# adityabalu/DiffNet

Hardware: AMD Instinct MI355X
Metric: elements*gauss_pts/sec (FEM loss+grad) (higher is better)
Workload: dtype f32; 1 GPU; 2-D Poisson energy loss + gradient wrt u, Q1, 512^2 nodes, 3^2 Gauss pts, batch 64/GPU, nu+f nodal fields, Dirichlet mask on all boundary faces held as one bit per node and sample (a general mask array), fused single pass (BASELINE.json configs[1] mesh); every step evaluates the next of 4 different batches in rotation (nu, f and the mask stream from HBM with non-temporal loads; of the 4 x 67 MB of; batch_per_gpu=64, parallelism=batch-sharded x1, batches_in_rotation=4, mask_format=bits

## Files before the change

diffnet_amd/csrc/dn_common.h:

```cpp
#pragma once
#include <hip/hip_runtime.h>
#include <stdint.h>

#include "../../include/diffnet_hip.h"

#define DN_WAVE 64

#define DN_LAUNCH_CHECK()                         \
    do {                                          \
        hipError_t e__ = hipGetLastError();       \
        if (e__ != hipSuccess) return (int)e__;   \
    } while (0)

namespace dn {

enum ConfigKey : int { CFG_PLAN2D = 0, CFG_PLAN3D, CFG_PLAN_FSDT, CFG_Q1_RULE_KERNEL, CFG_GPE_GATHER, CFG_GPE_TILED, CFG_Q1_3D_T16, CFG_Q1_3D_E1SUM, CFG_FSDT_GENERIC, CFG_Q1_3D_E1, CFG_HANDOVER_SPIN_LIMIT, CFG_CONV2D_V1, CFG_CONV_WRW_WGS, CFG_Q1_3D_N2, CFG_FSDT_FORM, CFG_COUNT };
const char* config(ConfigKey k);

__device__ __forceinline__ double wave_sum(double v) {
#pragma unroll
    for (int off = DN_WAVE / 2; off > 0; off >>= 1) v += __shfl_down(v, off, DN_WAVE);
    return v;
}

__device__ __forceinline__ double block_sum(double v, double* scratch, int tid, int nthreads) {
    v = wave_sum(v);
    const int lane = tid & (DN_WAVE - 1), wave = tid / DN_WAVE;
    if (lane == 0) scratch[wave] = v;
    __syncthreads();
    double r = 0.0;
    if (tid == 0) {
        const int nw = (nthreads + DN_WAVE - 1) / DN_WAVE;
        for (int w = 0; w < nw; ++w) r += scratch[w];
    }
    __syncthreads();
    return r;
}

__device__ __forceinline__ void block_sum2(double& a, double& b, double* scratch, int tid, int nthreads) {
    a = wave_sum(a);
    b = wave_sum(b);
    const int lane = tid & (DN_WAVE - 1), wave = tid / DN_WAVE;
    const int nw = (nthreads + DN_WAVE - 1) / DN_WAVE;
    if (lane == 0) { scratch[wave] = a; scratch[nw + wave] = b; }
    __syncthreads();
    double ra = 0.0, rb = 0.0;
    if (tid == 0) {
        for (int w = 0; w < nw; ++w) { ra += scratch[w]; rb += scratch[nw + w]; }
    }
    __syncthreads();
    a = ra; b = rb;
}

template <int N>
struct VecT;
template <>
struct VecT<1> { using type = float; };
template <>
struct VecT<2> { using type = float2; };
template <>
struct VecT<4> { using type = float4; };

#ifndef DN_NT_STORES
#define DN_NT_STORES 0
#endif
template <typename V, typename T>
__device__ __forceinline__ V ld_at(const T* __restrict__ base, unsigned index) {
    return *reinterpret_cast<const V*>(reinterpret_cast<const char*>(base) + (index * (unsigned)sizeof(T)));
}
template <typename V, typename T>
__device__ __forceinline__ void st_at(T* __restrict__ base, unsigned index, const V& v) {
#if DN_NT_STORES
    char* a = reinterpret_cast<char*>(base) + (index * (unsigned)sizeof(T));
    if constexpr (sizeof(V) == 16) {
        typedef float v4f __attribute__((ext_vector_type(4)));
        __builtin_nontemporal_store(__builtin_bit_cast(v4f, v), reinterpret_cast<v4f*>(a));
    } else if constexpr (sizeof(V) == 8) {
        typedef float v2f __attribute__((ext_vector_type(2)));
        __builtin_nontemporal_store(__builtin_bit_cast(v2f, v), reinterpret_cast<v2f*>(a));
    } else {
        __builtin_nontemporal_store(v, reinterpret_cast<V*>(a));
    }
#else
    *reinterpret_cast<V*>(reinterpret_cast<char*>(base) + (index * (unsigned)sizeof(T))) = v;
#endif
}

template <int NW, bool VEC, typename T>
__device__ __forceinline__ void load_seg(const T* __restrict__ base, unsigned rowoff, int x0, int nx, T (&dst)[NW + 1]) {
    if constexpr (VEC && (NW == 2 || NW == 4)) {
        const unsigned xl = (unsigned)min(x0, nx - NW);
        if constexpr (sizeof(T) == 4) {
            using V = typename VecT<NW>::type;
            const V v = ld_at<V>(base, rowoff + xl);
            const T* vf = reinterpret_cast<const T*>(&v);
#pragma unroll
            for (int k = 0; k < NW; ++k) dst[k] = vf[k];
        } else {
            static_assert(sizeof(T) == 1, "load_seg: 1- or 4-byte elements");
            if constexpr (NW == 4) {
                const uint32_t w = ld_at<uint32_t>(base, rowoff + xl);
#pragma unroll
                for (int k = 0; k < 4; ++k) dst[k] = (T)((w >> (8 * k)) & 0xffu);
            } else {
                const uint16_t w = ld_at<uint16_t>(base, rowoff + xl);
                dst[0] = (T)(w & 0xffu);
                dst[1] = (T)(w >> 8);
            }
        }
    } else {
#pragma unroll
        for (int k = 0; k < NW; ++k) dst[k] = ld_at<T>(base, rowoff + (unsigned)min(x0 + k, nx - 1));
    }
    dst[NW] = ld_at<T>(base, rowoff + (unsigned)min(x0 + NW, nx - 1));
}

template <int NW, bool VEC, typename T>
__device__ __forceinline__ void load_seg_stream(const T* __restrict__ base, unsigned rowoff, int x0, int nx, T (&dst)[NW + 1]) {
    if constexpr (VEC && NW == 4 && sizeof(T) == 4) {
        typedef T v4t __attribute__((ext_vector_type(4)));
        const unsigned xl = (unsigned)min(x0, nx - NW);
        const v4t v = __builtin_nontemporal_load(reinterpret_cast<const v4t*>(reinterpret_cast<const char*>(base) + (rowoff + xl) * 4u));
        dst[0] = v.x; dst[1] = v.y; dst[2] = v.z; dst[3] = v.w;
        dst[NW] = ld_at<T>(base, rowoff + (unsigned)min(x0 + NW, nx - 1));
    } else if constexpr (VEC && NW == 4 && sizeof(T) == 1) {
        const unsigned xl = (unsigned)min(x0, nx - NW);
        const uint32_t w = __builtin_nontemporal_load(reinterpret_cast<const uint32_t*>(reinterpret_cast<const char*>(base) + (rowoff + xl)));
#pragma unroll
        for (int k = 0; k < 4; ++k) dst[k] = (T)((w >> (8 * k)) & 0xffu);
        dst[NW] = ld_at<T>(base, rowoff + (unsigned)min(x0 + NW, nx - 1));
    } else {
        load_seg<NW, VEC>(base, rowoff, x0, nx, dst);
    }
}

template <int NW, bool VEC, typename T>
__device__ __forceinline__ void load_own(const T* __restrict__ base, unsigned rowoff, int x0, int nx, T (&dst)[NW]) {
    if constexpr (VEC && (NW == 2 || NW == 4)) {
        const unsigned xl = (unsigned)min(x0, nx - NW);
        if constexpr (sizeof(T) == 4) {
            using V = typename VecT<NW>::type;
            const V v = ld_at<V>(base, rowoff + xl);
            const T* vf = reinterpret_cast<const T*>(&v);
#pragma unroll
            for (int k = 0; k < NW; ++k) dst[k] = vf[k];
        } else {
            if constexpr (NW == 4) {
                const uint32_t w = ld_at<uint32_t>(base, rowoff + xl);
#pragma unroll
                for (int k = 0; k < 4; ++k) dst[k] = (T)((w >> (8 * k)) & 0xffu);
            } else {
                const uint16_t w = ld_at<uint16_t>(base, rowoff + xl);
                dst[0] = (T)(w & 0xffu);
                dst[1] = (T)(w >> 8);
            }
        }
    } else {
#pragma unroll
        for (int k = 0; k < NW; ++k) dst[k] = ld_at<T>(base, rowoff + (unsigned)min(x0 + k, nx - 1));
    }
}

template <int NW, bool VEC>
__device__ __forceinline__ void store_seg(float* __restrict__ base, unsigned rowoff, int x0, int nx, const float (&src)[NW]) {
    if constexpr (VEC && (NW == 2 || NW == 4)) {
        if (x0 + NW <= nx) {
            using V = typename VecT<NW>::type;
            V v;
            float* vf = reinterpret_cast<float*>(&v);
#pragma unroll
            for (int k = 0; k < NW; ++k) vf[k] = src[k];
            st_at<V>(base, rowoff + (unsigned)x0, v);
        }
    } else {
#pragma unroll
        for (int k = 0; k < NW; ++k)
            if (x0 + k < nx) st_at<float>(base, rowoff + (unsigned)(x0 + k), src[k]);
    }
}

}
```

diffnet_amd/csrc/poisson2d_q1_cf.hip:

```cpp
#include <cstdlib>
#include <type_traits>

#define DN_NT_STORES 1
#include "poisson_common.h"

namespace dn {

enum : int { CF_NU = 1, CF_F = 2, CF_BC = 8, CF_BC_U8C = 16, CF_BC_PACKED = 32, CF_PK_NB1 = 64, CF_PK_NB2 = 128, CF_UA = 256, CF_ONE = 512 };

template <int E>
struct CfRow {
    float u[E + 1], n[E + 1], f[E + 1];
    float g[E + 1];
    float du[E], pn[E];
    float keep[E];
    float keepx;
    BcRaw<E> bc;
    uint32_t m8[2][2];
    uint32_t mb[2];
    uint32_t bx[2];
};

constexpr int CF_W = 4;
constexpr int CF_TS = 128;
constexpr int CF_NSLOT = 64;
constexpr unsigned CF_SPIN_MAX = 1u << 20;

__device__ __forceinline__ unsigned lds_addr(const void* p) { return (unsigned)(uintptr_t)(__attribute__((address_space(3))) const void*)p; }
__device__ __forceinline__ void lds_st(unsigned a, float v) { asm volatile("ds_write_b32 %0, %1" ::"v"(a), "v"(v) : "memory"); }
__device__ __forceinline__ void lds_st(unsigned a, unsigned v) { asm volatile("ds_write_b32 %0, %1" ::"v"(a), "v"(v) : "memory"); }
__device__ __forceinline__ void lds_ld_nowait(float& d, unsigned a) { asm volatile("ds_read_b32 %0, %1" : "=v"(d) : "v"(a) : "memory"); }
__device__ __forceinline__ unsigned lds_ld_u(unsigned a) {
    unsigned d;
    asm volatile("ds_read_b32 %0, %1\n\ts_waitcnt lgkmcnt(0)" : "=v"(d) : "v"(a) : "memory");
    return d;
}
__device__ __forceinline__ float lds_ld(unsigned a) {
    float d;
    asm volatile("ds_read_b32 %0, %1\n\ts_waitcnt lgkmcnt(0)" : "=v"(d) : "v"(a) : "memory");
    return d;
}
template <int N>
__device__ __forceinline__ void lds_wait(float (&v)[N]) {
    if constexpr (N == 5) asm volatile("s_waitcnt lgkmcnt(0)" : "+v"(v[0]), "+v"(v[1]), "+v"(v[2]), "+v"(v[3]), "+v"(v[4])::"memory");
    else if constexpr (N == 4) asm volatile("s_waitcnt lgkmcnt(0)" : "+v"(v[0]), "+v"(v[1]), "+v"(v[2]), "+v"(v[3])::"memory");
    else if constexpr (N == 3) asm volatile("s_waitcnt lgkmcnt(0)" : "+v"(v[0]), "+v"(v[1]), "+v"(v[2])::"memory");
    else if constexpr (N == 2) asm volatile("s_waitcnt lgkmcnt(0)" : "+v"(v[0]), "+v"(v[1])::"memory");
    else { static_assert(N == 1, "lds_wait: 1..5 values"); asm volatile("s_waitcnt lgkmcnt(0)" : "+v"(v[0])::"memory"); }
}

template <int E, bool VEC, int FL, int W>
__global__ void __launch_bounds__(W > 1 ? CF_TS * W : 256, W > 1 ? 4 : 2) poisson2d_q1_cf_kernel(const PoissonParams p) {
    constexpr int NW = E;
    constexpr bool HAS_NU = (FL & CF_NU) != 0, HAS_F = (FL & CF_F) != 0;
    constexpr bool BC_ANY = (FL & (CF_BC | CF_BC_U8C | CF_BC_PACKED)) != 0, BC_U8C = (FL & CF_BC_U8C) != 0, BC_PACKED = (FL & CF_BC_PACKED) != 0;
    constexpr bool UA = (FL & CF_UA) != 0, ONE = (FL & CF_ONE) != 0;
    static_assert(!ONE || ((BC_PACKED || BC_U8C) && (FL & CF_PK_NB2) == 0), "CF_ONE: one packed or uint8-constant condition");
    static_assert(!UA || (E == 4 && VEC && W == 1), "CF_UA: four elements per thread, vector accesses, one strip per workgroup");
    const int T = W > 1 ? CF_TS : (int)blockDim.x;
    const int sub = W > 1 ? __builtin_amdgcn_readfirstlane((int)threadIdx.x / CF_TS) : 0;
    const int tid = W > 1 ? (int)threadIdx.x - sub * CF_TS : (int)threadIdx.x;
    const int chunk = blockIdx.x, strip = W > 1 ? (int)blockIdx.y * W + sub : selected_strip(p, (int)blockIdx.y), b = blockIdx.z;
    const bool active = W == 1 || strip < p.nstrips;
    const bool chain_dn = W > 1 && sub > 0;
    const bool chain_up = W > 1 && sub + 1 < W && strip + 1 < p.nstrips;
    const int q = chunk * (T - 1) + tid;
    const int ex0 = q * E;
    const int x0 = ex0;
    const bool col_owner = !(chunk > 0 && tid == 0);
    const bool lastcol = UA && x0 + NW == p.nx - 1;
    const int64_t nps = (int64_t)p.nx * p.ny;
    const SampleBases sb = sample_bases(p, b, nps);
    const int R = p.rows_per_strip;
    const int sb0 = strip * R, sc0 = min(sb0 + R, p.nely);
    const int ey_begin = (sb0 > 0 && !chain_dn) ? sb0 - 1 : sb0;
    const int ey_end = sc0;
    const int r_from = sb0;
    const int e_from = sb0, e_until = p.nely;
    const bool top_row = sc0 == p.nely;

    __shared__ float xch[2][256];
    __shared__ double red[W > 1 ? 4 * W : 8];
    __shared__ int last_flag;
    constexpr int CW = W > 1 ? W : 2, SEAM_WORDS = 6 * (E + 1);
    __shared__ float cf_edge[W > 1 ? W : 1][W > 1 ? CF_NSLOT : 1];
    __shared__ unsigned cf_xflag[W > 1 ? W : 1];
    __shared__ float cf_seam[CW - 1][W > 1 ? SEAM_WORDS : 1][W > 1 ? CF_TS : 1];
    __shared__ unsigned cf_sflag[CW - 1][2][2];
    const int lane = tid & 63, wv = __builtin_amdgcn_readfirstlane(tid >> 6);
    unsigned seq = 0u;
    if constexpr (W > 1) {
        static_assert(CF_TS == 128, "two waves per sub-strip");
        if (threadIdx.x < (unsigned)W) cf_xflag[threadIdx.x] = 0u;
        if (threadIdx.x < 4u * (W - 1)) (&cf_sflag[0][0][0])[threadIdx.x] = 0u;
        __syncthreads();
    }
    if ((blockIdx.x | blockIdx.y | blockIdx.z) == 0u) fold_prev_sums(p, (int)threadIdx.x, (int)blockDim.x, red);
    float spin_poison = 0.f;
    auto spin_until = [&](const unsigned* flag, unsigned want) {
        const unsigned fa = lds_addr(flag);
        const unsigned lim = p.spin_limit > 0 ? (unsigned)p.spin_limit : CF_SPIN_MAX;
        unsigned n = 0;
        for (; n < lim; ++n) {
            if ((unsigned)__builtin_amdgcn_readfirstlane((int)lds_ld_u(fa)) >= want) break;
            __builtin_amdgcn_s_sleep(1);
        }
        if (n == lim) spin_poison = __builtin_nanf("");
    };

    const bool has_mask[2] = {sb.mask[0] != nullptr, sb.mask[1] != nullptr};
    const uint8_t* mask8[2];
    mask8[0] = reinterpret_cast<const uint8_t*>(has_mask[0] ? sb.mask[0] : sb.mask[1]);
    mask8[1] = reinterpret_cast<const uint8_t*>(has_mask[1] ? sb.mask[1] : sb.mask[0]);

    constexpr unsigned NBITS = (1u << (NW + 1)) - 1u;
    constexpr int NB = !BC_PACKED ? 0 : ((FL & CF_PK_NB2) ? 2 : ((FL & CF_PK_NB1) ? 1 : 0));
    const bool isbits[2] = {p.bc[0].kind == DN_MASK_BITS, p.bc[1].kind == DN_MASK_BITS};
    const unsigned bsel[2] = {isbits[0] ? NBITS : 0u, isbits[1] ? NBITS : 0u};
    const int src0 = (NB == 2 || isbits[0]) ? 0 : 1;
    const int kone = p.bc[0].kind >= 0 ? 0 : 1;
    const uint32_t* bptr[2] = {reinterpret_cast<const uint32_t*>(sb.mask[src0]), reinterpret_cast<const uint32_t*>(sb.mask[1])};
    const unsigned brow[2] = {(unsigned)p.bc[src0].row_bytes / 4u, (unsigned)p.bc[1].row_bytes / 4u};
    unsigned bw0[2], bw1[2];
#pragma unroll
    for (int j = 0; j < 2; ++j) {
        const int rw = max((int)brow[j], 1);
        bw0[j] = (unsigned)min(x0 >> 5, rw - 1);
        bw1[j] = (unsigned)min((x0 >> 5) + 1, rw - 1);
    }
    const unsigned bsh = (unsigned)x0 & 31u;
    unsigned boxx[2] = {0u, 0u};
#pragma unroll
    for (int k = 0; k < 2; ++k) {
        const int faces = p.bc[k].kind == DN_MASK_BOX ? p.bc[k].box_faces : 0;
#pragma unroll
        for (int n = 0; n <= NW; ++n) {
            const bool on = ((faces & DN_FACE_XLO) && x0 + n == 0) || ((faces & DN_FACE_XHI) && x0 + n == p.nx - 1);
            boxx[k] |= on ? (1u << n) : 0u;
        }
    }
    const int ylo[2] = {(p.bc[0].kind == DN_MASK_BOX && (p.bc[0].box_faces & DN_FACE_YLO)) ? 0 : -1,
                        (p.bc[1].kind == DN_MASK_BOX && (p.bc[1].box_faces & DN_FACE_YLO)) ? 0 : -1};
    const int yhi[2] = {(p.bc[0].kind == DN_MASK_BOX && (p.bc[0].box_faces & DN_FACE_YHI)) ? p.ny - 1 : -1,
                        (p.bc[1].kind == DN_MASK_BOX && (p.bc[1].box_faces & DN_FACE_YHI)) ? p.ny - 1 : -1};
    auto packed_issue = [&](int yc, CfRow<E>& r) {
#pragma unroll
        for (int j = 0; j < NB; ++j) {
            const unsigned ro = (unsigned)yc * brow[j];
            const uint32_t w0 = ld_at<uint32_t>(bptr[j], ro + bw0[j]), w1 = ld_at<uint32_t>(bptr[j], ro + bw1[j]);
            r.mb[j] = __builtin_amdgcn_alignbit(w1, w0, bsh);
        }
        if constexpr (ONE) {
            if constexpr (NB == 0) r.bx[0] = (yc == (kone ? ylo[1] : ylo[0]) || yc == (kone ? yhi[1] : yhi[0])) ? NBITS : (kone ? boxx[1] : boxx[0]);
        } else {
#pragma unroll
            for (int k = 0; k < 2; ++k) r.bx[k] = (yc == ylo[k] || yc == yhi[k]) ? NBITS : boxx[k];
        }
    };

    auto row_issue = [&](int yr, CfRow<E>& r) {
        const int yp = min(yr, p.ny - 1);
        const unsigned rowoff = (unsigned)yp * (unsigned)p.nx;
        load_seg<NW, VEC>(sb.u, rowoff, x0, p.nx, r.u);
        if constexpr (HAS_NU) load_seg_stream<NW, VEC>(sb.nu, rowoff, x0, p.nx, r.n);
        if constexpr (HAS_F) load_seg_stream<NW, VEC>(sb.f, rowoff, x0, p.nx, r.f);
        if constexpr (BC_PACKED) {
            packed_issue(yp, r);
        } else if constexpr (BC_U8C && ONE) {
            uint8_t t[NW + 1];
            load_seg_stream<NW, VEC>(mask8[0], rowoff, x0, p.nx, t);
            uint32_t w = 0u;
#pragma unroll
            for (int n = 0; n < NW; ++n) w |= (uint32_t)t[n] << (8 * n);
            r.m8[0][0] = w;
            r.m8[0][1] = t[NW];
        } else if constexpr (BC_U8C) {
#pragma unroll
            for (int k = 0; k < 2; ++k) {
                if (has_mask[k]) {
                    uint8_t t[NW + 1];
                    load_seg_stream<NW, VEC>(mask8[k], rowoff, x0, p.nx, t);
                    uint32_t w = 0u;
#pragma unroll
                    for (int n = 0; n < NW; ++n) w |= (uint32_t)t[n] << (8 * n);
                    r.m8[k][0] = w;
                    r.m8[k][1] = t[NW];
                }
            }
        } else if constexpr (BC_ANY) {
            bc_issue<NW, VEC>(p, sb, rowoff, x0, r.bc);
        }
    };
    auto row_bc = [&](CfRow<E>& r) {
#pragma unroll
        for (int n = 0; n < NW; ++n) r.keep[n] = 1.f;
        if constexpr (UA) r.keepx = 1.f;
        if constexpr ((BC_PACKED || BC_U8C) && ONE) {
            const float v = kone ? p.bc[1].value : p.bc[0].value;
            unsigned b = 0u;
            if constexpr (BC_PACKED) b = NB == 1 ? r.mb[0] : r.bx[0];
#pragma unroll
            for (int n = 0; n <= NW; ++n) {
                bool set;
                if constexpr (BC_PACKED) set = (b & (1u << n)) != 0u;
                else set = n < NW ? ((r.m8[0][0] >> (8 * n)) & 0xffu) != 0u : r.m8[0][1] != 0u;
                r.u[n] = set ? v : r.u[n];
                if (n < NW) r.keep[n] = set ? 0.f : 1.f;
                else if constexpr (UA) r.keepx = set ? 0.f : 1.f;
            }
        } else if constexpr (BC_PACKED) {
            unsigned b0 = r.bx[0], b1 = r.bx[1];
            if constexpr (NB == 2) { b0 |= r.mb[0] & bsel[0]; b1 |= r.mb[1] & bsel[1]; }
            if constexpr (NB == 1) { b0 |= r.mb[0] & bsel[0]; b1 |= r.mb[0] & bsel[1]; }
            const float v0 = p.bc[0].value, v1 = p.bc[1].value;
#pragma unroll
            for (int n = 0; n <= NW; ++n) {
                r.u[n] = (b0 & (1u << n)) ? v0 : r.u[n];
                r.u[n] = (b1 & (1u << n)) ? v1 : r.u[n];
                if (n < NW) r.keep[n] = ((b0 | b1) & (1u << n)) ? 0.f : 1.f;
            }
            if constexpr (UA) r.keepx = ((b0 | b1) & (1u << NW)) ? 0.f : 1.f;
        } else if constexpr (BC_U8C) {
#pragma unroll
            for (int k = 0; k < 2; ++k) {
                if (has_mask[k]) {
                    const float val = p.bc[k].value;
#pragma unroll
                    for (int n = 0; n <= NW; ++n) {
                        const bool set = has_mask[k] && (n < NW ? ((r.m8[k][0] >> (8 * n)) & 0xffu) != 0u : r.m8[k][1] != 0u);
                        r.u[n] = set ? val : r.u[n];
                        if (n < NW) r.keep[n] = set ? 0.f : r.keep[n];
                        else if constexpr (UA) r.keepx = set ? 0.f : r.keepx;
                    }
                }
            }
        } else if constexpr (BC_ANY) {
            if constexpr (UA) {
                float k5[NW + 1];
                bc_apply_all<NW>(p, sb, r.bc, r.u, k5);
#pragma unroll
                for (int n = 0; n < NW; ++n) r.keep[n] = k5[n];
                r.keepx = k5[NW];
            } else {
                bc_apply<NW>(p, sb, r.bc, r.u, r.keep);
            }
        }
    };

    float e1_acc = 0.f, e2_acc = 0.f, sq_acc = 0.f;
    int par = 0;

    float pend_v[NW];
    unsigned pend_row = 0u;
    bool pend_st = false;
    float pend_x = 0.f;
    auto flush_store = [&]() {
        if (pend_st) store_seg<NW, VEC>(sb.out, pend_row, x0, p.nx, pend_v);
        if constexpr (UA) {
            if (pend_st && lastcol) st_at<float>(sb.out, pend_row + (unsigned)(p.nx - 1), pend_x);
        }
        pend_st = false;
    };
    auto emit_row = [&](const float (&o)[NW + 1], const float (&keep)[NW], int yr, bool owned_row, float keepx = 1.f) {
        float left;
        if constexpr (W > 1) {
            const float up = __shfl_up(o[NW], 1, 64);
            const unsigned ea = lds_addr(&cf_edge[sub][seq & (CF_NSLOT - 1)]);
            float edge = 0.f;
            if (wv == 0) {
                if (lane == 63) { lds_st(ea, o[NW]); lds_st(lds_addr(&cf_xflag[sub]), seq + 1u); }
            } else {
                spin_until(&cf_xflag[sub], seq + 1u);
                edge = lds_ld(ea);
            }
            left = lane > 0 ? up : edge;
            ++seq;
        } else {
            xch[par][tid] = o[NW];
            asm volatile("s_waitcnt lgkmcnt(0)\n\ts_barrier" ::: "memory");
            left = (tid > 0) ? xch[par][tid - 1] : 0.f;
            par ^= 1;
        }
        const bool st = owned_row && col_owner && (!UA || x0 + NW <= p.nx - 1);
#pragma unroll
        for (int n = 0; n < NW; ++n) {
            const float t = (o[n] + (n == 0 ? left : 0.f)) * keep[n];
            sq_acc = st ? fmaf(t, t, sq_acc) : sq_acc;
            pend_v[n] = t * p.out_scale;
            if constexpr (W > 1) pend_v[n] += spin_poison;
        }
        if constexpr (UA) {
            const float t = o[NW] * keepx;
            sq_acc = (st && lastcol) ? fmaf(t, t, sq_acc) : sq_acc;
            pend_x = t * p.out_scale;
        }
        pend_row = (unsigned)yr * (unsigned)p.nx;
        pend_st = st && sb.out != nullptr;
        flush_store();
    };

    const float mx0 = p.T.mxs[0], mx1 = p.T.mxs[1], mx2 = p.T.mxs[2], mx3 = p.T.mxs[3];
    const float my0 = p.T.m[0], my1 = p.T.m[1], my2 = p.T.m[2], my3 = p.T.m[3];
    const float k0 = p.T.q1c[0], k1 = p.T.q1c[1], h0 = p.T.q1c[2], h1 = p.T.q1c[3], nb = -p.T.beta;
    constexpr bool ROWSTAGED = (FL & CF_BC) == 0, STAGE_DU = W == 1;
    const float xm[4] = {p.T.q1xm[0], p.T.q1xm[1], p.T.q1xm[2], p.T.q1xm[3]}, ym[4] = {p.T.q1ym[0], p.T.q1ym[1], p.T.q1ym[2], p.T.q1ym[3]};
    const float px0 = p.T.q1px[0], px1 = p.T.q1px[1], sy0 = p.T.q1sy[0], sy1 = p.T.q1sy[1];

    constexpr bool FMASS = HAS_F && ROWSTAGED;
    const float cx00 = p.T.q1mx[0], cx01 = p.T.q1mx[1], cx11 = p.T.q1mx[2], cy00 = p.T.q1my[0], cy01 = p.T.q1my[1], cy11 = p.T.q1my[2];
    const float alpha = p.T.alpha;
    auto fstage = [&](CfRow<E>& r) {
        if constexpr (FMASS) {
#pragma unroll
            for (int n = 0; n <= NW; ++n) r.g[n] = 0.f;
#pragma unroll
            for (int e = 0; e < E; ++e) {
                if (ex0 + e < p.nelx) {
                    r.g[e] = fmaf(cx01, r.f[e + 1], fmaf(cx00, r.f[e], r.g[e]));
                    r.g[e + 1] = fmaf(cx11, r.f[e + 1], cx01 * r.f[e]);
                }
            }
        }
    };

    auto sstage = [&](CfRow<E>& r) {
        if constexpr (ROWSTAGED) {
#pragma unroll
            for (int e = 0; e < E; ++e) {
                if constexpr (HAS_NU) {
                    q1cf_stage(px0, px1, r.u[e], r.u[e + 1], r.n[e], r.n[e + 1], r.du[e], r.pn[e]);
                } else {
                    r.du[e] = r.u[e + 1] - r.u[e];
                    r.pn[e] = mx0;
                }
            }
        }
    };

    auto layer = [&](auto fresh, int ey, const CfRow<E>& L, CfRow<E>& U, const float (&cin)[NW + 1], float (&cout)[NW + 1]) {
        const bool own_layer = ey >= e_from && ey <= e_until;
        const float cnt = (own_layer && col_owner) ? 1.f : 0.f;
        if constexpr (decltype(fresh)::value) { row_bc(U); fstage(U); }
        sstage(U);
        float o[NW + 1], le1 = 0.f, le2 = 0.f;
#pragma unroll
        for (int n = 0; n <= NW; ++n) { o[n] = cin[n]; cout[n] = 0.f; }
        if constexpr (FMASS) {
#pragma unroll
            for (int n = 0; n <= NW; ++n) {
                const float tlo = fmaf(cy01, U.g[n], cy00 * L.g[n]), tup = fmaf(cy11, U.g[n], cy01 * L.g[n]);
                o[n] = fmaf(nb, tlo, o[n]);
                cout[n] = nb * tup;
                le2 = fmaf(U.u[n], tup, fmaf(L.u[n], tlo, le2));
            }
        }
        if constexpr (ROWSTAGED) {
            float V[NW + 1], S[NW + 1];
#pragma unroll
            for (int n = 0; n <= NW; ++n) {
                V[n] = U.u[n] - L.u[n];
                S[n] = HAS_NU ? fmaf(sy1, U.n[n], sy0 * L.n[n]) : my0;
            }
#pragma unroll
            for (int e = 0; e < E; ++e) {
                if (ex0 + e < p.nelx) {
                    const float a = STAGE_DU ? L.du[e] : L.u[e + 1] - L.u[e], b = STAGE_DU ? U.du[e] : U.u[e + 1] - U.u[e];
                    q1cf_elem(xm, ym, a, b, L.pn[e], U.pn[e], V[e], V[e + 1], S[e], S[e + 1], alpha, o[e], o[e + 1], cout[e], cout[e + 1], le1);
                }
            }
        } else {
#pragma unroll
            for (int e = 0; e < E; ++e) {
                if (ex0 + e < p.nelx) {
                    const float U0 = L.u[e], UX = L.u[e + 1] - L.u[e], UY = U.u[e] - L.u[e], UXY = (U.u[e + 1] - U.u[e]) - UX;
                    float P = mx0, Q = 0.f, Pp = my0, Qp = 0.f;
                    if constexpr (HAS_NU) {
                        const float N0 = L.n[e], NX = L.n[e + 1] - N0, NY = U.n[e] - N0, NXY = (U.n[e + 1] - U.n[e]) - NX;
                        P = fmaf(mx1, NX, mx0 * N0);
                        Q = fmaf(mx1, NXY, mx0 * NY);
                        Pp = fmaf(my1, NY, my0 * N0);
                        Qp = fmaf(my1, NXY, my0 * NX);
                    }
                    const float A0 = fmaf(Q, my1, P * my0), A1 = fmaf(Q, my2, P * my1), A2 = fmaf(Q, my3, P * my2);
                    const float B0 = fmaf(Qp, mx1, Pp * mx0), B1 = fmaf(Qp, mx2, Pp * mx1), B2 = fmaf(Qp, mx3, Pp * mx2);
                    const float tX0 = fmaf(UXY, A1, UX * A0), tX1 = fmaf(UXY, A2, UX * A1);
                    const float tY0 = fmaf(UXY, B1, UY * B0), tY1 = fmaf(UXY, B2, UY * B1);
                    le1 += fmaf(h1, fmaf(UXY, tY1, UY * tY0), h0 * fmaf(UXY, tX1, UX * tX0));
                    float cU0 = 0.f, cUX = k0 * tX0, cUY = k1 * tY0, cUXY = fmaf(k0, tX1, k1 * tY1);
                    if constexpr (HAS_F) {
                        const float F0 = L.f[e], FX = L.f[e + 1] - F0, FY = U.f[e] - F0, FXY = (U.f[e + 1] - U.f[e]) - FX;
                        const float S0 = fmaf(mx1, FX, mx0 * F0), S1 = fmaf(mx1, FXY, mx0 * FY);
                        const float T0 = fmaf(mx2, FX, mx1 * F0), T1 = fmaf(mx2, FXY, mx1 * FY);
                        const float L0 = fmaf(my1, S1, my0 * S0), LX = fmaf(my1, T1, my0 * T0);
                        const float LY = fmaf(my2, S1, my1 * S0), LXY = fmaf(my2, T1, my1 * T0);
                        le2 += fmaf(LXY, UXY, fmaf(LY, UY, fmaf(LX, UX, L0 * U0)));
                        cU0 = nb * L0;
                        cUX = fmaf(nb, LX, cUX);
                        cUY = fmaf(nb, LY, cUY);
                        cUXY = fmaf(nb, LXY, cUXY);
                    }
                    const float g01 = cUX - cUXY, g10 = cUY - cUXY;
                    o[e] += (cU0 - cUX) - g10;
                    o[e + 1] += g01;
                    cout[e] += g10;
                    cout[e + 1] += cUXY;
                }
            }
        }
        e1_acc = fmaf(cnt, le1, e1_acc);
        e2_acc = fmaf(cnt, le2, e2_acc);
        if (W > 1 && chain_dn && ey == sb0) {
            const unsigned s0 = lds_addr(&cf_seam[W > 1 ? sub - 1 : 0][0][tid]);
#pragma unroll
            for (int n = 0; n <= NW; ++n) lds_st(s0 + (4 * NW + 4 + n) * CF_TS * 4, o[n]);
#pragma unroll
            for (int n = 0; n < NW; ++n) lds_st(s0 + (5 * NW + 5 + n) * CF_TS * 4, L.keep[n]);
        } else {
            emit_row(o, L.keep, ey, ey >= r_from, L.keepx);
        }
    };
    auto publish_row = [&](const CfRow<E>& r) {
        const unsigned s0 = lds_addr(&cf_seam[W > 1 ? sub - 1 : 0][0][tid]);
#pragma unroll
        for (int n = 0; n <= NW; ++n) {
            lds_st(s0 + n * CF_TS * 4, r.u[n]);
            if constexpr (HAS_NU) lds_st(s0 + (NW + 1 + n) * CF_TS * 4, r.n[n]);
            if constexpr (FMASS) lds_st(s0 + (2 * NW + 2 + n) * CF_TS * 4, r.g[n]);
            else if constexpr (HAS_F) lds_st(s0 + (2 * NW + 2 + n) * CF_TS * 4, r.f[n]);
        }
        if (lane == 0) lds_st(lds_addr(&cf_sflag[W > 1 ? sub - 1 : 0][0][wv]), 1u);
    };
    auto fetch_row = [&](CfRow<E>& r) {
        spin_until(&cf_sflag[sub][0][wv], 1u);
        const unsigned s0 = lds_addr(&cf_seam[sub][0][tid]);
#pragma unroll
        for (int n = 0; n <= NW; ++n) lds_ld_nowait(r.u[n], s0 + n * CF_TS * 4);
        lds_wait(r.u);
        if constexpr (HAS_NU) {
#pragma unroll
            for (int n = 0; n <= NW; ++n) lds_ld_nowait(r.n[n], s0 + (NW + 1 + n) * CF_TS * 4);
            lds_wait(r.n);
        }
        if constexpr (FMASS) {
#pragma unroll
            for (int n = 0; n <= NW; ++n) lds_ld_nowait(r.g[n], s0 + (2 * NW + 2 + n) * CF_TS * 4);
            lds_wait(r.g);
        } else if constexpr (HAS_F) {
#pragma unroll
            for (int n = 0; n <= NW; ++n) lds_ld_nowait(r.f[n], s0 + (2 * NW + 2 + n) * CF_TS * 4);
            lds_wait(r.f);
        }
    };
    auto publish_carry = [&](const float (&c)[NW + 1]) {
        const unsigned s0 = lds_addr(&cf_seam[sub][0][tid]);
#pragma unroll
        for (int n = 0; n <= NW; ++n) lds_st(s0 + (3 * NW + 3 + n) * CF_TS * 4, c[n]);
        if (lane == 0) lds_st(lds_addr(&cf_sflag[sub][1][wv]), 1u);
    };

    auto set_prio = [&](int e) {
        switch (((ey_end - e) >> 1) & 3) {
            case 0: __builtin_amdgcn_s_setprio(0); break;
            case 1: __builtin_amdgcn_s_setprio(1); break;
            case 2: __builtin_amdgcn_s_setprio(2); break;
            default: __builtin_amdgcn_s_setprio(3); break;
        }
    };

    constexpr std::true_type FRESH{};
    constexpr std::false_type LANDED{};
    if (active) {
    CfRow<E> RA, RB;
    float carryA[NW + 1], carryB[NW + 1];
#pragma unroll
    for (int n = 0; n <= NW; ++n) carryA[n] = carryB[n] = 0.f;
    row_issue(ey_begin, RA);
    row_bc(RA);
    fstage(RA);
    sstage(RA);
    if constexpr (W > 1) {
        if (chain_dn) publish_row(RA);
    }
    int ey = ey_begin;
    bool odd = false;
    const int n_main = chain_up ? ey_end - 1 : ey_end;
    for (; ey + 1 < n_main; ey += 2) {
        set_prio(ey);
        row_issue(ey + 1, RB);
        layer(FRESH, ey, RA, RB, carryA, carryB);
        row_issue(ey + 2, RA);
        layer(FRESH, ey + 1, RB, RA, carryB, carryA);
    }
    if (ey < n_main) {
        set_prio(ey);
        row_issue(ey + 1, RB);
        layer(FRESH, ey, RA, RB, carryA, carryB);
        odd = true;
        ++ey;
    }
    if constexpr (W > 1) {
        if (chain_up) {
            __builtin_amdgcn_s_setprio(0);
            if (odd) { fetch_row(RA); layer(LANDED, ey, RB, RA, carryB, carryA); publish_carry(carryA); }
            else { fetch_row(RB); layer(LANDED, ey, RA, RB, carryA, carryB); publish_carry(carryB); }
        }
    }
    if (top_row) {
        float o[NW + 1], keep[NW];
#pragma unroll
        for (int n = 0; n <= NW; ++n) o[n] = odd ? carryB[n] : carryA[n];
#pragma unroll
        for (int n = 0; n < NW; ++n) keep[n] = odd ? RB.keep[n] : RA.keep[n];
        emit_row(o, keep, p.ny - 1, true, odd ? RB.keepx : RA.keepx);
        flush_store();
    }
    if constexpr (W > 1) {
        if (chain_dn) {
            spin_until(&cf_sflag[sub - 1][1][wv], 1u);
            const unsigned s0 = lds_addr(&cf_seam[sub - 1][0][tid]);
            float o[NW + 1], cy[NW + 1], keep[NW];
#pragma unroll
            for (int n = 0; n <= NW; ++n) lds_ld_nowait(o[n], s0 + (4 * NW + 4 + n) * CF_TS * 4);
            lds_wait(o);
#pragma unroll
            for (int n = 0; n <= NW; ++n) lds_ld_nowait(cy[n], s0 + (3 * NW + 3 + n) * CF_TS * 4);
            lds_wait(cy);
#pragma unroll
            for (int n = 0; n < NW; ++n) lds_ld_nowait(keep[n], s0 + (5 * NW + 5 + n) * CF_TS * 4);
            lds_wait(keep);
#pragma unroll
            for (int n = 0; n <= NW; ++n) o[n] += cy[n];
            emit_row(o, keep, sb0, true);
            flush_store();
        }
    }
    }

    if constexpr (W > 1) {
        e1_acc += spin_poison;
        sq_acc += spin_poison;
        if (spin_poison != spin_poison && p.counter != nullptr && (threadIdx.x & 63u) == 0u) atomicOr(p.counter + DN_WS_ERRWORD, 1u);
    }
    if (p.want_sums) finish_sums(p, e1_acc, e2_acc, sq_acc, (int)threadIdx.x, (int)blockDim.x, red, &last_flag);
}

template <int E, bool VEC, int FL>
static void cf_launch_one(const PoissonParams& pp, const Geom2D& g, int batch, hipStream_t s) {
    if constexpr (E == 4 && VEC && (FL & CF_UA) == 0) {
        if (g.W == CF_W) {
            hipLaunchKernelGGL((poisson2d_q1_cf_kernel<E, VEC, FL, CF_W>), dim3(g.chunks, (g.strips + CF_W - 1) / CF_W, batch),
                               dim3(CF_TS * CF_W), 0, s, pp);
            return;
        }
    }
    hipLaunchKernelGGL((poisson2d_q1_cf_kernel<E, VEC, FL, 1>), dim3(g.chunks, g.strips, batch), dim3(g.T), 0, s, pp);
}

template <int E, bool VEC, int UAF = 0>
static void cf_launch_flags(const PoissonParams& pp, const Geom2D& g, int batch, hipStream_t s) {
    const bool any = pp.bc[0].kind >= 0 || pp.bc[1].kind >= 0;
    bool u8c = any, packed = false;
    for (int k = 0; k < 2; ++k) {
        if (pp.bc[k].kind >= 0 && (!pp.bc[k].mask_is_u8 || pp.bc[k].field)) u8c = false;
        if (pp.bc[k].kind == DN_MASK_BITS || pp.bc[k].kind == DN_MASK_BOX) packed = true;
    }
    const int nbits = (pp.bc[0].kind == DN_MASK_BITS) + (pp.bc[1].kind == DN_MASK_BITS);
    const bool one = (pp.bc[0].kind >= 0) != (pp.bc[1].kind >= 0);
    const int nf = (pp.nu ? CF_NU : 0) | (pp.f ? CF_F : 0);
#define DN_CF(FLAGS)                                                                         \
    (!any ? cf_launch_one<E, VEC, (FLAGS) | UAF>(pp, g, batch, s)                                  \
          : packed ? (nbits == 2 ? cf_launch_one<E, VEC, (FLAGS) | UAF | CF_BC_PACKED | CF_PK_NB2>(pp, g, batch, s)          \
                     : nbits == 1 ? (one ? cf_launch_one<E, VEC, (FLAGS) | UAF | CF_BC_PACKED | CF_PK_NB1 | CF_ONE>(pp, g, batch, s)        \
                                         : cf_launch_one<E, VEC, (FLAGS) | UAF | CF_BC_PACKED | CF_PK_NB1>(pp, g, batch, s))        \
                     : one ? cf_launch_one<E, VEC, (FLAGS) | UAF | CF_BC_PACKED | CF_ONE>(pp, g, batch, s)                   \
                           : cf_launch_one<E, VEC, (FLAGS) | UAF | CF_BC_PACKED>(pp, g, batch, s))                   \
          : u8c ? (one ? cf_launch_one<E, VEC, (FLAGS) | UAF | CF_BC_U8C | CF_ONE>(pp, g, batch, s)                \
                       : cf_launch_one<E, VEC, (FLAGS) | UAF | CF_BC_U8C>(pp, g, batch, s))                \
                : cf_launch_one<E, VEC, (FLAGS) | UAF | CF_BC>(pp, g, batch, s))
    switch (nf) {
        case 0: DN_CF(0); break;
        case CF_NU: DN_CF(CF_NU); break;
        case CF_F: DN_CF(CF_F); break;
        default: DN_CF(CF_NU | CF_F); break;
    }
#undef DN_CF
}

int poisson2d_q1_cf_chain() { return CF_W; }

int launch_poisson2d_q1_cf(const PoissonParams& pp, const Geom2D& g, int batch, bool vec, hipStream_t s) {
    if (g.W > 1 && !(g.W == poisson2d_q1_cf_chain() && g.E == 4 && vec && g.T == CF_TS && g.R + 3 <= CF_NSLOT)) return DN_E_BADARG;
    if (g.ua) {
        if (g.E != 4 || g.W != 1 || (pp.nx & 3) != 1 || pp.nx < 9) return DN_E_BADARG;
        cf_launch_flags<4, true, CF_UA>(pp, g, batch, s);
        return 0;
    }
    if (g.E == 4 && vec) { cf_launch_flags<4, true>(pp, g, batch, s); return 0; }
    if (g.E == 2 && vec) { cf_launch_flags<2, true>(pp, g, batch, s); return 0; }
    if (g.E == 2) { cf_launch_flags<2, false>(pp, g, batch, s); return 0; }
    return DN_E_UNSUPPORTED;
}

}
```

Baseline: 2634 billion elements*gauss_pts/s.

## Share halo column via DPP lane exchange and stream interior u rows nontemporally

When the kernel runs with one wave per strip, four-wide vectors and no boundary-condition flag, each lane now takes its right-neighbour halo value (the fifth element) for u, nu and f from the next lane's first vector element through a DPP row shift. Only the last lane, or a lane with no neighbour, keeps its own scalar load, and that load is redirected to a single wave-uniform address. This is meant to cut redundant scalar gather traffic per row. Interior row pairs also load u with nontemporal loads, while the first and last trips keep plain loads, presumably so halo rows shared with adjacent strips stay cached. The risk is that DPP row_shr works within 16-lane rows, so lanes at row boundaries may receive wrong values. The extra code may also add register pressure.

After: 2806 billion elements*gauss_pts/s, median of 6. 1.07x the previous value.

```diff
diff --git a/diffnet_amd/csrc/dn_common.h b/diffnet_amd/csrc/dn_common.h
--- a/diffnet_amd/csrc/dn_common.h
+++ b/diffnet_amd/csrc/dn_common.h
@@ -134,6 +134,22 @@
     }
 }
 
+template <bool NT>
+__device__ __forceinline__ void load_seg4_xs(const float* __restrict__ base, unsigned rowoff, int x0, int nx, unsigned xs, float (&dst)[5]) {
+    typedef float v4t __attribute__((ext_vector_type(4)));
+    const unsigned xl = (unsigned)min(x0, nx - 4);
+    const v4t* a = reinterpret_cast<const v4t*>(reinterpret_cast<const char*>(base) + (rowoff + xl) * 4u);
+    v4t v;
+    if constexpr (NT) v = __builtin_nontemporal_load(a);
+    else v = *a;
+    dst[0] = v.x; dst[1] = v.y; dst[2] = v.z; dst[3] = v.w;
+    dst[4] = ld_at<float>(base, rowoff + xs);
+}
+__device__ __forceinline__ void seg_take_shared(float (&dst)[5], bool has_nb) {
+    const int t = __builtin_amdgcn_update_dpp(__builtin_bit_cast(int, dst[4]), __builtin_bit_cast(int, dst[0]), 0x130, 0xf, 0xf, false);
+    dst[4] = has_nb ? __builtin_bit_cast(float, t) : dst[4];
+}
+
 template <int NW, bool VEC, typename T>
 __device__ __forceinline__ void load_own(const T* __restrict__ base, unsigned rowoff, int x0, int nx, T (&dst)[NW]) {
     if constexpr (VEC && (NW == 2 || NW == 4)) {
diff --git a/diffnet_amd/csrc/poisson2d_q1_cf.hip b/diffnet_amd/csrc/poisson2d_q1_cf.hip
--- a/diffnet_amd/csrc/poisson2d_q1_cf.hip
+++ b/diffnet_amd/csrc/poisson2d_q1_cf.hip
@@ -69,6 +69,9 @@
     const int x0 = ex0;
     const bool col_owner = !(chunk > 0 && tid == 0);
     const bool lastcol = UA && x0 + NW == p.nx - 1;
+    constexpr bool XCH = W == 1 && VEC && E == 4 && (FL & CF_BC) == 0;
+    const bool has_nb = XCH && ((int)threadIdx.x & 63) < 63 && (int)threadIdx.x + 1 < (int)blockDim.x && !lastcol;
+    const unsigned xs = (unsigned)min((has_nb ? __builtin_amdgcn_readfirstlane(q) + 63 : q) * E + NW, p.nx - 1);
     const int64_t nps = (int64_t)p.nx * p.ny;
     const SampleBases sb = sample_bases(p, b, nps);
     const int R = p.rows_per_strip;
@@ -158,12 +161,18 @@
         }
     };
 
-    auto row_issue = [&](int yr, CfRow<E>& r) {
+    auto row_issue = [&](auto nt_u, int yr, CfRow<E>& r) {
         const int yp = min(yr, p.ny - 1);
         const unsigned rowoff = (unsigned)yp * (unsigned)p.nx;
-        load_seg<NW, VEC>(sb.u, rowoff, x0, p.nx, r.u);
-        if constexpr (HAS_NU) load_seg_stream<NW, VEC>(sb.nu, rowoff, x0, p.nx, r.n);
-        if constexpr (HAS_F) load_seg_stream<NW, VEC>(sb.f, rowoff, x0, p.nx, r.f);
+        if constexpr (XCH) {
+            load_seg4_xs<decltype(nt_u)::value>(sb.u, rowoff, x0, p.nx, xs, r.u);
+            if constexpr (HAS_NU) load_seg4_xs<true>(sb.nu, rowoff, x0, p.nx, xs, r.n);
+            if constexpr (HAS_F) load_seg4_xs<true>(sb.f, rowoff, x0, p.nx, xs, r.f);
+        } else {
+            load_seg<NW, VEC>(sb.u, rowoff, x0, p.nx, r.u);
+            if constexpr (HAS_NU) load_seg_stream<NW, VEC>(sb.nu, rowoff, x0, p.nx, r.n);
+            if constexpr (HAS_F) load_seg_stream<NW, VEC>(sb.f, rowoff, x0, p.nx, r.f);
+        }
         if constexpr (BC_PACKED) {
             packed_issue(yp, r);
         } else if constexpr (BC_U8C && ONE) {
@@ -192,6 +201,11 @@
         }
     };
     auto row_bc = [&](CfRow<E>& r) {
+        if constexpr (XCH) {
+            seg_take_shared(r.u, has_nb);
+            if constexpr (HAS_NU) seg_take_shared(r.n, has_nb);
+            if constexpr (HAS_F) seg_take_shared(r.f, has_nb);
+        }
 #pragma unroll
         for (int n = 0; n < NW; ++n) r.keep[n] = 1.f;
         if constexpr (UA) r.keepx = 1.f;
@@ -337,7 +351,7 @@
         }
     };
 
-    auto layer = [&](auto fresh, int ey, const CfRow<E>& L, CfRow<E>& U, const float (&cin)[NW + 1], float (&cout)[NW + 1]) {
+    auto layer = [&](auto fresh, int ey, const CfRow<E>& L, CfRow<E>& U, const float (&cin)[NW + 1], float (&cout)[NW + 1]) __attribute__((always_inline)) {
         const bool own_layer = ey >= e_from && ey <= e_until;
         const float cnt = (own_layer && col_owner) ? 1.f : 0.f;
         if constexpr (decltype(fresh)::value) { row_bc(U); fstage(U); }
@@ -474,7 +488,9 @@
     float carryA[NW + 1], carryB[NW + 1];
 #pragma unroll
     for (int n = 0; n <= NW; ++n) carryA[n] = carryB[n] = 0.f;
-    row_issue(ey_begin, RA);
+    constexpr std::true_type NT_U{};
+    constexpr std::false_type PLAIN_U{};
+    row_issue(PLAIN_U, ey_begin, RA);
     row_bc(RA);
     fstage(RA);
     sstage(RA);
@@ -484,16 +500,30 @@
     int ey = ey_begin;
     bool odd = false;
     const int n_main = chain_up ? ey_end - 1 : ey_end;
-    for (; ey + 1 < n_main; ey += 2) {
+    auto trip2 = [&](auto nt_u) __attribute__((always_inline)) {
         set_prio(ey);
-        row_issue(ey + 1, RB);
+        row_issue(nt_u, ey + 1, RB);
         layer(FRESH, ey, RA, RB, carryA, carryB);
-        row_issue(ey + 2, RA);
+        row_issue(nt_u, ey + 2, RA);
         layer(FRESH, ey + 1, RB, RA, carryB, carryA);
+        ey += 2;
+    };
+    if constexpr (XCH) {
+        if (ey + 1 < n_main) trip2(PLAIN_U);
+        while (ey + 3 < n_main) trip2(NT_U);
+        if (ey + 1 < n_main) trip2(PLAIN_U);
+    } else {
+        for (; ey + 1 < n_main; ey += 2) {
+            set_prio(ey);
+            row_issue(PLAIN_U, ey + 1, RB);
+            layer(FRESH, ey, RA, RB, carryA, carryB);
+            row_issue(PLAIN_U, ey + 2, RA);
+            layer(FRESH, ey + 1, RB, RA, carryB, carryA);
+        }
     }
     if (ey < n_main) {
         set_prio(ey);
-        row_issue(ey + 1, RB);
+        row_issue(PLAIN_U, ey + 1, RB);
         layer(FRESH, ey, RA, RB, carryA, carryB);
         odd = true;
         ++ey;
```
